# erwincoumans/tiny-differentiable-simulator

Measured on AMD Instinct MI355X. Metric: env-steps/sec, higher is better.
Workload: dtype f64

## Files before the change

### tiny-differentiable-simulator_amd/csrc/tds_oct.hip

```cpp
#include <hip/hip_runtime.h>
#include <stdlib.h>

#include "tds_device_model.h"
#include "tds_kernels.h"
#include "tds_lanes.h"
#include "tds_oct_windows.h"
#include "tds_step_shared.h"

#ifdef TDS_OCT_PROF
#ifndef TDS_OCT_PROF_WG
#define TDS_OCT_PROF_WG 3
#endif
__device__ unsigned long long tds_oct_prof_buf[64];
__device__ unsigned long long tds_oct_prof_clk[64];
__device__ unsigned long long tds_oct_prof_wg[3 * 2048];
__device__ int tds_oct_prof_iter = 500;
#define OCT_STAMP(k, pin)                                                                       \
  do {                                                                                          \
    unsigned long long t_;                                                                      \
    auto p_ = (pin);        \
    asm volatile("s_memtime %0\n\ts_waitcnt lgkmcnt(0)" : "=s"(t_), "+v"(p_)::"memory");        \
    if (prof_on) prof_t[k] = t_;                                                                \
  } while (0)
#define OCT_BAR_T(k)       \
  do {                     \
    OCT_STAMP(k, tid);     \
    OCT_BAR();             \
    OCT_STAMP((k) + 1, tid); \
  } while (0)
#define OCT_BAR_W(k, first)                                                                     \
  do {                                                                                          \
    unsigned long long a_, b_;                                                                  \
    asm volatile("s_memtime %0\n\ts_waitcnt lgkmcnt(0)" : "=s"(a_), "+v"(tid)::"memory");       \
    OCT_BAR();                                                                                  \
    asm volatile("s_memtime %0\n\ts_waitcnt lgkmcnt(0)" : "=s"(b_), "+v"(tid)::"memory");       \
    if (prof_on && (first)) {                                                                   \
      prof_t[k] = a_;                                                                           \
      prof_t[(k) + 1] = b_;                                                                     \
    } else if (prof_on) {                                                                       \
      prof_t[(k) + 2] += b_ - a_;                                                               \
    }                                                                                           \
  } while (0)
#else
#define OCT_STAMP(k, pin) do { } while (0)
#define OCT_BAR_T(k) OCT_BAR()
#define OCT_BAR_W(k, first) OCT_BAR()
#endif

#ifdef TDS_OCT_MARKS
#define OCT_MARK(name) asm volatile("; OCTMARK " name ::: "memory")
#else
#define OCT_MARK(name) do { } while (0)
#endif

namespace {

#define OCT_SYNC()                                             \
  do {                                                         \
    __builtin_amdgcn_fence(__ATOMIC_ACQ_REL, "wavefront");     \
    __builtin_amdgcn_wave_barrier();                           \
  } while (0)

template <int CTRL>
__device__ __forceinline__ double oct_dpp(double v) {
  const int l = __double2loint(v), h = __double2hiint(v);
  const int lo = __builtin_amdgcn_update_dpp(0, l, CTRL, 0xF, 0xF, true);
  const int hi = __builtin_amdgcn_update_dpp(0, h, CTRL, 0xF, 0xF, true);
  return __hiloint2double(hi, lo);
}
template <int CTRL>
__device__ __forceinline__ float oct_dpp(float v) {
  return __int_as_float(__builtin_amdgcn_update_dpp(0, __float_as_int(v), CTRL, 0xF, 0xF, true));
}
template <typename T>
__device__ __forceinline__ T pair_other(T v) { return oct_dpp<0xB1>(v); }
template <int K, typename T>
__device__ __forceinline__ T pair_bcast(T v) { return oct_dpp<(K == 0 ? 0xA0 : 0xF5)>(v); }
template <typename T>
__device__ __forceinline__ T oct_sum(T v) {
  asm volatile("" : "+v"(v));
  v += oct_dpp<0xB1>(v);
  v += oct_dpp<0x4E>(v);
  v += oct_dpp<0x141>(v);
  return v;
}
template <int K>
__device__ __forceinline__ double oct_bcast(double v) {
  const double t = __builtin_amdgcn_update_dpp(0.0, v, 0x150 + K, 0xF, 0x3, false);
  return __builtin_amdgcn_update_dpp(t, v, 0x150 + 8 + K, 0xF, 0xC, false);
}
template <int K>
__device__ __forceinline__ float oct_bcast(float v) {
  const int b = __float_as_int(v);
  const int t = __builtin_amdgcn_update_dpp(0, b, 0x150 + K, 0xF, 0x3, false);
  return __int_as_float(__builtin_amdgcn_update_dpp(t, b, 0x150 + 8 + K, 0xF, 0xC, false));
}

struct OctOff {
  int lcw, legf, swl, qdp, fac, win, xs, cp, stride;
};
struct OctLds {
  static constexpr int LCW = 6;
  static constexpr int ZW = 14;
  static constexpr int Z_B = 10, Z_A = 11, Z_G = 12, Z_HL = 13;
  static constexpr int NCP = 17;
};
__host__ __device__ inline OctOff oct_layout(int in_dim) {
  OctOff o;
  int at = in_dim + 4;
  at = (at + 1) & ~1;
  o.lcw = at;  at += 8 * OctLds::LCW;
  o.legf = at; at += 4 * 3;
  o.swl = at;  at += 8 * 6;
  o.qdp = at;  at += 8;
  o.fac = at;  at += 28;
  o.win = at;  at += 2 * 8 * OctLds::ZW;
  o.xs = at;   at += 3 * OctLds::NCP + 1;
  o.cp = at;   at += 5 * OctLds::NCP + 1;
  at = (at + 1) & ~1;
  while ((((at * 2) & 63) % 8) != 0 || ((at * 2) & 63) == 0 || ((at * 2) & 63) == 32) at += 2;
  o.stride = at;
  return o;
}

struct OctKernArgs {
  const void *mdl, *x_in;
  void *y_out;
  const void *actions;
  void *x_feedback, *obs_out;
  TdsStepCtl ctl;
  int n_envs;
  OctOff O;
};
using TB = TdsOctTab;
constexpr int TDS_OCT_PRIO = 1;

#define OCT_ST(v, p) (*(p) = (v))
#define OCT_BAR()                                                                        \
  do {                                                                                   \
    if constexpr (W2) asm volatile("s_waitcnt lgkmcnt(0)\n\ts_barrier" ::: "memory");    \
    else OCT_SYNC();                                                                     \
  } while (0)

template <typename T, typename TR, bool LOOP, int BUILD>
__device__ __forceinline__ void oct_body(const DevModel<T> *__restrict__ mdl_arg, const TR *x_in, TR *__restrict__ y_out,
                                         const TR *__restrict__ actions, TR *x_feedback ,
                                         TR *__restrict__ obs_out, const TdsStepCtl &ctl_arg, int n_envs, const OctOff &O) {
  extern __shared__ __align__(16) unsigned char tds_oct_smem[];
  T *const sm = reinterpret_cast<T *>(tds_oct_smem);
#ifdef TDS_OCT_PROF
  if (threadIdx.x == 0 && blockIdx.x < 2048) {
    unsigned long long c_;
    asm volatile("s_memrealtime %0\n\ts_waitcnt lgkmcnt(0)" : "=s"(c_)::"memory");
    tds_oct_prof_wg[3 * blockIdx.x] = c_;
  }
#endif
  constexpr bool W2 = BUILD >= 2;
  constexpr bool BATCH_SCHUR = LOOP && BUILD == 3;
  constexpr int nq = 14, nd = 14, adim = 8, in_dim = nq + nd + adim + 3, w_obs = nq + nd + 2;
  constexpr int NT = W2 ? 128 : 64;
  T *const CT = sm + 8 * O.stride;
  {
    const int t = threadIdx.x;
    constexpr int TN = (TB::TOTAL + NT - 1) / NT, XN = (in_dim + 7) / 8;
    T tv[TN], xv[XN];
#pragma unroll
    for (int k = 0; k < TN; ++k) {
      const int i = t + k * NT;
      tv[k] = i < TB::TOTAL ? mdl_arg->oct_tab[i] : T(0);
    }
    const int lane0 = t & 7, grp0 = (t & 63) >> 3, env0 = blockIdx.x * 8 + grp0;
    const bool valid0 = env0 < n_envs && t < 64;
#pragma unroll
    for (int k = 0; k < XN; ++k) {
      const int i = lane0 + 8 * k;
      const bool act = actions != nullptr && i >= nq + nd && i < nq + nd + adim;
      xv[k] = (!valid0 || i >= in_dim) ? T(0) : act ? (T)actions[(size_t)env0 * adim + (i - nq - nd)] : (T)x_in[(size_t)env0 * in_dim + i];
    }
#pragma unroll
    for (int k = 0; k < TN; ++k) {
      const int i = t + k * NT;
      if (i < TB::TOTAL) CT[i] = tv[k];
    }
    if (t < 64) {
      T *const xr = sm + grp0 * O.stride;
#pragma unroll
      for (int k = 0; k < XN; ++k) {
        const int i = lane0 + 8 * k;
        if (i < in_dim) xr[i] = xv[k];
      }
      if (lane0 < 4) xr[in_dim + lane0] = T(0);
    }
    if constexpr (W2) __syncthreads();
    else OCT_SYNC();
  }
  const int nsteps = LOOP ? ctl_arg.nsub : 1;
  T next_act = T(0);
  int act_blk = 0, y_slot = 0, o_slot = 0;
  if constexpr (LOOP) {
    if (ctl_arg.act_pool != nullptr && ctl_arg.act_blocks > 0) act_blk = (ctl_arg.act_first + 1) % ctl_arg.act_blocks;
    if (ctl_arg.y_ring != nullptr && ctl_arg.y_slots > 0) y_slot = ctl_arg.y_first % ctl_arg.y_slots;
    if (ctl_arg.obs_ring != nullptr && ctl_arg.obs_slots > 0) o_slot = ctl_arg.obs_first % ctl_arg.obs_slots;
  }
  const int act_slot = (int)(CT + (threadIdx.x & 7) * TB::LSTR)[TB::ACT];
  for (int it = 0; it < nsteps; ++it) {
  const __attribute__((address_space(4))) char *ka_seg = (const __attribute__((address_space(4))) char *)__builtin_amdgcn_kernarg_segment_ptr();
  int tid = threadIdx.x;
  if constexpr (LOOP) asm volatile("" : "+s"(ka_seg), "+v"(tid));
  const int wv = W2 ? __builtin_amdgcn_readfirstlane(tid >> 6) : 0;
  const bool is_main = !W2 || wv == 0, is_help = !W2 || wv == 1;
  if constexpr (W2 && TDS_OCT_PRIO != 0) {
    if (BUILD != 4 && wv == 0) __builtin_amdgcn_s_setprio(3);
    else __builtin_amdgcn_s_setprio(0);
  }
  (void)is_main;
  (void)is_help;
#ifdef TDS_OCT_PROF
  unsigned long long prof_t[56] = {};
  const bool prof_on = blockIdx.x == TDS_OCT_PROF_WG && it == tds_oct_prof_iter;
  if (it == 0 && tid == 0 && blockIdx.x < 2048) {
    unsigned long long c_;
    asm volatile("s_memrealtime %0\n\ts_waitcnt lgkmcnt(0)" : "=s"(c_)::"memory");
    tds_oct_prof_wg[3 * blockIdx.x + 1] = c_;
  }
  if (blockIdx.x == TDS_OCT_PROF_WG && it < 32 && tid == 0) {
    unsigned long long c0_, c1_;
    asm volatile("s_memtime %0\n\ts_memrealtime %1\n\ts_waitcnt lgkmcnt(0)" : "=s"(c0_), "=s"(c1_)::"memory");
    tds_oct_prof_clk[2 * it] = c0_;
    tds_oct_prof_clk[2 * it + 1] = c1_;
  }
#endif
  const int lane = tid & 7;
  const int grp = (tid & 63) >> 3;
  const int env = blockIdx.x * 8 + grp;
  const bool valid = env < n_envs;
  T *const E = sm + grp * O.stride;
  T *const xr = E;
  const int leg = lane >> 1, pos = lane & 1;
  const int dq = 6 + lane;
  const T *const CL = CT + lane * TB::LSTR;
  typename TdsCtlRef<LOOP>::type ctl = TdsCtlRef<LOOP>::get(ctl_arg, ka_seg + __builtin_offsetof(OctKernArgs, ctl));
  const T dt = CT[TB::SC + TB::DT];
  const int pgs_iters = (int)CT[TB::SC + TB::PGS_ITERATIONS];
  const bool last = it == nsteps - 1;
  OCT_STAMP(0, tid);

  T q, qd, tau;
  T Sl[6], R[9], p[3], sw[6], v[6], a0[6];
  T R5[9], P[3], A4[3], A5[3], pA3[3], pA4[3], pA5[3], v5[6], a5[6];
  T Lc[6], l10, id0, id1, sq0, sq1, my_id, my_sq, Ls[15], ids[6], sq_ids[6], qd_new, qdr_new[6];
  T Cb, Cr[6], It[10];
  T u = T(0), urm = T(0);
  T u_init = T(0), urm_init = T(0);
  T sw_mu = T(0), sw_rest = T(0), sw_cap = T(0), sw_hip = T(0);
  int na = 0, NA = 0;

  auto root_frame = [&](T sx, T cx, T sy, T cy, T sz, T cz) {
    R5[0] = cy * cz;                 R5[1] = -cy * sz;                R5[2] = sy;
    R5[3] = sx * sy * cz + cx * sz;  R5[4] = cx * cz - sx * sy * sz;  R5[5] = -sx * cy;
    R5[6] = sx * sz - cx * sy * cz;  R5[7] = cx * sy * sz + sx * cz;  R5[8] = cx * cy;
    P[0] = xr[0] + CT[TB::SC + TB::BASE_T];
    P[1] = xr[1] + CT[TB::SC + TB::BASE_T + 1];
    P[2] = xr[2] + CT[TB::SC + TB::BASE_T + 2];
    A4[0] = T(0); A4[1] = cx; A4[2] = sx;
    A5[0] = sy; A5[1] = -sx * cy; A5[2] = cx * cy;
    pA3[0] = T(0); pA3[1] = P[2]; pA3[2] = -P[1];
    cross3(P, A4, pA4);
    cross3(P, A5, pA5);
  };
  auto times_inertia = [&](const T *I, const T *s, T *F) {
    T t3[3];
    sym3_mulv(I, s, F);
    cross3(I + 6, s + 3, t3);
    F[0] += t3[0];
    F[1] += t3[1];
    F[2] += t3[2];
    cross3(I + 6, s, t3);
    F[3] = I[9] * s[3] - t3[0];
    F[4] = I[9] * s[4] - t3[1];
    F[5] = I[9] * s[5] - t3[2];
  };
  auto dot6 = [&](const T *a, const T *b) -> T { return dot3(a, b) + dot3(a + 3, b + 3); };

  auto main_kin = [&]() {
    OCT_MARK("main_top");
    q = xr[dq];
    qd = xr[nq + dq];
    tau = T(0);
    {
      const int act_i = act_slot;
      if (act_i >= 0) {
        const int var = nq + nd + adim;
        const T kp = xr[var], kd = xr[var + 1], max_force = xr[var + 2];
        const T act_lim = CT[TB::SC + TB::ACTION_LIMIT];
        T a = xr[nq + nd + act_i];
        a = a < act_lim ? a : act_lim;
        a = a > -act_lim ? a : -act_lim;
        const T q_des = CL[TB::IPOSE] + a;
        T f = kp * (q_des - q) + kd * (T(0) - qd);
        f = f > -max_force ? f : -max_force;
        f = f < max_force ? f : max_force;
        tau = f;
      }
      tau -= CL[TB::STIFF] * q + CL[TB::DAMP] * qd;
      asm volatile("" : "+v"(tau));
    }
    OCT_MARK("main_jcalc");
#pragma unroll
    for (int k = 0; k < 6; ++k) Sl[k] = CL[TB::S + k];
    T Rp[9], tp[3];
    {
      T sn, cs;
      tds_sincos(q * CL[TB::ROTF], &sn, &cs);
      const T c1 = T(1) - cs;
      const T nx = CL[TB::NAX], ny = CL[TB::NAX + 1], nz = CL[TB::NAX + 2];
      T RJ[9];
      RJ[0] = cs + c1 * CL[TB::NN + 0];
      RJ[1] = c1 * CL[TB::NN + 1] - sn * nz;
      RJ[2] = c1 * CL[TB::NN + 2] + sn * ny;
      RJ[3] = c1 * CL[TB::NN + 1] + sn * nz;
      RJ[4] = cs + c1 * CL[TB::NN + 3];
      RJ[5] = c1 * CL[TB::NN + 4] - sn * nx;
      RJ[6] = c1 * CL[TB::NN + 2] - sn * ny;
      RJ[7] = c1 * CL[TB::NN + 4] + sn * nx;
      RJ[8] = cs + c1 * CL[TB::NN + 5];
      const T tJ[3] = {Sl[3] * q, Sl[4] * q, Sl[5] * q};
      if (CT[TB::SC + TB::XT_IDENT] != T(0)) {
#pragma unroll
        for (int k = 0; k < 9; ++k) Rp[k] = RJ[k];
#pragma unroll
        for (int k = 0; k < 3; ++k) tp[k] = CL[TB::XT + 9 + k] + tJ[k];
      } else {
        T RT[9], r[3];
#pragma unroll
        for (int k = 0; k < 9; ++k) RT[k] = CL[TB::XT + k];
        mat3_mul(RT, RJ, Rp);
        mat3_mulv(RT, tJ, r);
#pragma unroll
        for (int k = 0; k < 3; ++k) tp[k] = CL[TB::XT + 9 + k] + r[k];
      }
    }
    OCT_MARK("main_rootsincos");
    {
      T rs, rc;
      tds_sincos(xr[3 + (lane < 3 ? lane : 0)], &rs, &rc);
      const T sx = oct_bcast<0>(rs), cx = oct_bcast<0>(rc);
      const T sy = oct_bcast<1>(rs), cy = oct_bcast<1>(rc);
      const T sz = oct_bcast<2>(rs), cz = oct_bcast<2>(rc);
      if constexpr (W2) {
        if (lane < 3) {
          T *const sc = E + O.win + 8 * OctLds::ZW + 96;
          sc[2 * lane] = rs;
          sc[2 * lane + 1] = rc;
        }
      }
      root_frame(sx, cx, sy, cy, sz, cz);
    }
    OCT_MARK("main_rootvel");
    {
      const T d0 = xr[nq + 0], d1 = xr[nq + 1], d2 = xr[nq + 2], d3 = xr[nq + 3], d4 = xr[nq + 4], d5 = xr[nq + 5];
      const T U[3] = {d0, d1, d2};
      const T J3[3] = {d3, T(0), T(0)}, J4[3] = {A4[0] * d4, A4[1] * d4, A4[2] * d4}, J5[3] = {A5[0] * d5, A5[1] * d5, A5[2] * d5};
      const T W4[3] = {J3[0] + J4[0], J3[1] + J4[1], J3[2] + J4[2]};
      const T W5[3] = {W4[0] + J5[0], W4[1] + J5[1], W4[2] + J5[2]};
      T pJ3[3], pJ4[3], pJ5[3];
      cross3(P, J3, pJ3);
      cross3(P, J4, pJ4);
      cross3(P, J5, pJ5);
      const T pW4[3] = {pJ3[0] + pJ4[0], pJ3[1] + pJ4[1], pJ3[2] + pJ4[2]};
      const T pW5[3] = {pW4[0] + pJ5[0], pW4[1] + pJ5[1], pW4[2] + pJ5[2]};
      const T V3[3] = {U[0] + pJ3[0], U[1] + pJ3[1], U[2] + pJ3[2]};
      const T V4[3] = {U[0] + pW4[0], U[1] + pW4[1], U[2] + pW4[2]};
      const T V5[3] = {U[0] + pW5[0], U[1] + pW5[1], U[2] + pW5[2]};
      T a45[3], a55[3], t1[3], t2[3], l3[3], l4[3], l5[3];
      cross3(J3, J4, a45);
      cross3(W4, J5, a55);
      cross3(J3, pJ3, t1);
      cross3(V3, J3, t2);
      l3[0] = t1[0] + t2[0]; l3[1] = t1[1] + t2[1]; l3[2] = t1[2] + t2[2];
      cross3(W4, pJ4, t1);
      cross3(V4, J4, t2);
      l4[0] = t1[0] + t2[0]; l4[1] = t1[1] + t2[1]; l4[2] = t1[2] + t2[2];
      cross3(W5, pJ5, t1);
      cross3(V5, J5, t2);
      l5[0] = t1[0] + t2[0]; l5[1] = t1[1] + t2[1]; l5[2] = t1[2] + t2[2];
#pragma unroll
      for (int k = 0; k < 3; ++k) {
        v5[k] = W5[k];
        v5[3 + k] = V5[k];
        a5[k] = a45[k] + a55[k];
        a5[3 + k] = (l3[k] + l4[k] + l5[k]) - CT[TB::SC + TB::GRAV + k];
      }
    }
    OCT_MARK("main_legs");
    {
      const bool take = pos == 1;
      T Rq[9], pq[3];
#pragma unroll
      for (int k = 0; k < 9; ++k) {
        const T sh = pair_bcast<0>(Rp[k]);
        Rq[k] = take ? sh : ((k == 0 || k == 4 || k == 8) ? T(1) : T(0));
      }
#pragma unroll
      for (int k = 0; k < 3; ++k) {
        const T sh = pair_bcast<0>(tp[k]);
        pq[k] = take ? sh : T(0);
      }
      T Rl[9], pl[3], r[3];
      mat3_mul(Rq, Rp, Rl);
      mat3_mulv(Rq, tp, r);
#pragma unroll
      for (int k = 0; k < 3; ++k) pl[k] = pq[k] + r[k];
      mat3_mul(R5, Rl, R);
      mat3_mulv(R5, pl, r);
      p[0] = P[0] + r[0];
      p[1] = P[1] + r[1];
      p[2] = P[2] + r[2];
      mat3_mulv(R, Sl, sw);
      mat3_mulv(R, Sl + 3, sw + 3);
      T c[3];
      cross3(p, sw, c);
      sw[3] += c[0];
      sw[4] += c[1];
      sw[5] += c[2];
      T vJ[6];
#pragma unroll
      for (int k = 0; k < 6; ++k) vJ[k] = sw[k] * qd;
#pragma unroll
      for (int k = 0; k < 6; ++k) {
        const T sh = pair_bcast<0>(vJ[k]);
        v[k] = v5[k] + (vJ[k] + (take ? sh : T(0)));
      }
      T cb[6];
      cross3(v, vJ, cb);
      T c1[3], c2[3];
      cross3(v, vJ + 3, c1);
      cross3(v + 3, vJ, c2);
      cb[3] = c1[0] + c2[0];
      cb[4] = c1[1] + c2[1];
      cb[5] = c1[2] + c2[2];
#pragma unroll
      for (int k = 0; k < 6; ++k) {
        const T sh = pair_bcast<0>(cb[k]);
        a0[k] = a5[k] + (cb[k] + (take ? sh : T(0)));
      }
    }
    OCT_MARK("main_publish_kin");
    {
      T *const swl = E + O.swl + lane * 6;
#pragma unroll
      for (int k = 0; k < 6; ++k) swl[k] = sw[k];
      if constexpr (W2) {
        T *const kin = E + O.win + 8 * OctLds::ZW + lane * 12;
#pragma unroll
        for (int k = 0; k < 9; ++k) kin[k] = R[k];
#pragma unroll
        for (int k = 0; k < 3; ++k) kin[9 + k] = p[k];
      }
    }
    OCT_MARK("main_kin_end");
    OCT_STAMP(1, sw[5]);
  };

  const int ystr = ctl.y_stride;
  const int out_dim = (int)CT[TB::SC + TB::OUTPUT_DIM];
  const int nv = (int)CT[TB::SC + TB::NUM_VISUALS];
  auto y_where = [&](TR *&yo, TR *&yo2, int &yend, int &yend2) {
    int ys = y_slot;
    asm volatile("" : "+s"(ys));
    yo = nullptr;
    yo2 = nullptr;
    yend = ystr;
    yend2 = out_dim;
    if (LOOP && ctl.y_ring != nullptr) {
      yo = tds_global((TR *)ctl.y_ring) + ((size_t)ys * ctl.ring_envs + env) * ystr;
      if (last && y_out != nullptr) yo2 = y_out + (size_t)env * out_dim;
    } else if (last && y_out != nullptr) {
      yo = y_out + (size_t)env * (LOOP ? out_dim : ystr);
      yend = LOOP ? out_dim : ystr;
    }
  };
  unsigned sig_tok = 0u;

  auto help_np = [&]() {
    OCT_MARK("help_np");
    if constexpr (LOOP) {
      if (it > 0 && ctl.obs_ring != nullptr && ctl.peer_arrive != nullptr)
        sig_tok = tds_peer_count_in(ctl, (o_slot == 0 ? ctl.obs_slots : o_slot) - 1);
      if (ctl.act_pool != nullptr && it + 1 < nsteps && valid)
        next_act = (T)tds_global((const TR *)ctl.act_pool)[((size_t)act_blk * ctl.act_envs + env) * adim + lane];
    }
    if constexpr (W2) {
      const T *const kin = E + O.win + 8 * OctLds::ZW + lane * 12;
#pragma unroll
      for (int k = 0; k < 9; ++k) R[k] = kin[k];
#pragma unroll
      for (int k = 0; k < 3; ++k) p[k] = kin[9 + k];
      const T *const sc = E + O.win + 8 * OctLds::ZW + 96;
      root_frame(sc[0], sc[1], sc[2], sc[3], sc[4], sc[5]);
    }
    {
      T *const cpx = E + O.cp;
      const T n[3] = {CT[TB::SC + TB::PLANE_N], CT[TB::SC + TB::PLANE_N + 1], CT[TB::SC + TB::PLANE_N + 2]};
      const T pc = CT[TB::SC + TB::PLANE_C];
      auto sphere = [&](const T *Rl, const T *pl, const T *loc, T rad, T *pt, T &dist) {
        T ctr[3];
        mat3_mulv(Rl, loc, ctr);
        ctr[0] += pl[0];
        ctr[1] += pl[1];
        ctr[2] += pl[2];
        const T t = -((-dot3(ctr, n)) + pc);
        dist = t - rad;
        pt[0] = ctr[0] - rad * n[0];
        pt[1] = ctr[1] - rad * n[1];
        pt[2] = ctr[2] - rad * n[2];
      };
      T pt0[3], pt1[3], ptt[3], d0, d1, dtt;
      sphere(R, p, CL + TB::CPL0, CL[TB::CPR0], pt0, d0);
      sphere(R, p, CL + TB::CPL1, CL[TB::CPR1], pt1, d1);
      sphere(R5, P, CT + TB::ROOT + TB::R_CPL, CT[TB::ROOT + TB::R_CPR], ptt, dtt);
      const bool act0 = valid && d0 < T(0), act1 = valid && d1 < T(0), actt = valid && dtt < T(0) && CT[TB::ROOT + TB::R_CPR] >= T(0);
      const unsigned long long b0 = __ballot(act0), b1 = __ballot(act1), bt = __ballot(actt);
      const unsigned m0 = (unsigned)((b0 >> (grp * 8)) & 0xFFull), m1 = (unsigned)((b1 >> (grp * 8)) & 0xFFull);
      const unsigned below = (1u << lane) - 1u;
      const int r0 = (actt ? 1 : 0) + __popc(m0 & below) + __popc(m1 & below);
      const int r1 = r0 + (act0 ? 1 : 0);
      if (act0) {
        cpx[0 * OctLds::NCP + r0] = pt0[0];
        cpx[1 * OctLds::NCP + r0] = pt0[1];
        cpx[2 * OctLds::NCP + r0] = pt0[2];
        cpx[3 * OctLds::NCP + r0] = d0;
        cpx[4 * OctLds::NCP + r0] = (T)lane;
      }
      if (act1) {
        cpx[0 * OctLds::NCP + r1] = pt1[0];
        cpx[1 * OctLds::NCP + r1] = pt1[1];
        cpx[2 * OctLds::NCP + r1] = pt1[2];
        cpx[3 * OctLds::NCP + r1] = d1;
        cpx[4 * OctLds::NCP + r1] = (T)lane;
      }
      if (actt && lane == 0) {
        cpx[0 * OctLds::NCP] = ptt[0];
        cpx[1 * OctLds::NCP] = ptt[1];
        cpx[2 * OctLds::NCP] = ptt[2];
        cpx[3 * OctLds::NCP] = dtt;
        cpx[4 * OctLds::NCP] = T(8);
      }
      na = (actt ? 1 : 0) + __popc(m0) + __popc(m1);
#pragma unroll
      for (int g = 0; g < 8; ++g) {
        const int c = __popc((unsigned)((b0 >> (g * 8)) & 0xFFull)) + __popc((unsigned)((b1 >> (g * 8)) & 0xFFull)) + (int)((bt >> (g * 8)) & 1ull);
        NA = c > NA ? c : NA;
      }
      if constexpr (W2) {
        if ((tid & 63) == 0) sm[in_dim + 3] = (T)NA;
      }
    }
    OCT_STAMP(8, na);
  };
  auto help_poses = [&]() {
    OCT_MARK("help_signal_poses");
    if constexpr (LOOP) {
      if (ctl.act_pool != nullptr && !last) xr[nq + nd + lane] = next_act;
      if (it > 0 && ctl.obs_ring != nullptr) {
        if (ctl.peer_arrive != nullptr) tds_peer_finish(ctl, (o_slot == 0 ? ctl.obs_slots : o_slot) - 1, sig_tok);
        else tds_signal_slot(ctl, (o_slot == 0 ? ctl.obs_slots : o_slot) - 1);
      }
    }
    TR *yo, *yo2;
    int yend, yend2;
    y_where(yo, yo2, yend, yend2);
    (void)yend;
    (void)yend2;
    if (valid && yo != nullptr && nv > 0) {
      auto pose_out = [&](const T *Rl, const T *pl, const T *vx, int k) {
        T Ro[9], po[3], qo[4];
        mat3_mul(Rl, vx, Ro);
        mat3_mulv(Rl, vx + 9, po);
        matrix_to_quat(Ro, qo);
        TR *o = yo + (nq + nd) + 7 * k;
        OCT_ST((TR)(pl[0] + po[0]), &o[0]);
        OCT_ST((TR)(pl[1] + po[1]), &o[1]);
// ... 397 lines not shown
#pragma unroll
      for (int c = 0; c < 6; ++c) {
        lch[c] = lcw[hl * OctLds::LCW + c];
        lca[c] = lcw[(hl + 1) * OctLds::LCW + c];
      }
      const T *const lf = E + O.legf + (hl >> 1) * 3;
      const T lf0 = lf[0], lf1 = lf[1], lf2 = lf[2];
      z1 -= lf0 * z0;
#pragma unroll
      for (int rr = 0; rr < 6; ++rr) rw.zr[rr] = rw.zr[rr] - (lch[rr] * z0 + lca[rr] * z1);
      rw.z0 = z0 * lf1;
      rw.z1 = z1 * lf2;
      row[0] = rw.z0;
      row[1] = rw.z1;
  };
  auto rows_park = [&](const RowRegs &rw) {
      T *const row = E + O.win + lane * OctLds::ZW;
#pragma unroll
      for (int rr = 0; rr < 6; ++rr) row[2 + rr] = rw.zr[rr];
  };
  auto rows_fetch = [&](RowRegs &rw) {
      const T *const row = E + O.win + lane * OctLds::ZW;
      rw.z0 = row[0];
      rw.z1 = row[1];
#pragma unroll
      for (int rr = 0; rr < 6; ++rr) rw.zr[rr] = row[2 + rr];
  };
  auto rows_root = [&](int bo, const RowRegs &rw) {
      OCT_MARK("rows_root");
      T *const row = E + O.win + bo + lane * OctLds::ZW;
      const T z0 = rw.z0, z1 = rw.z1;
      T zr[6];
#pragma unroll
      for (int rr = 0; rr < 6; ++rr) zr[rr] = rw.zr[rr];
      const bool real = rw.real;
      static_for<1, 6>([&](auto rc) {
        constexpr int rr = decltype(rc)::value;
        static_for<0, rr>([&](auto cc) {
          constexpr int c = decltype(cc)::value;
          zr[rr] -= Ls[(rr * (rr - 1)) / 2 + c] * zr[c];
        });
      });
#pragma unroll
      for (int rr = 0; rr < 6; ++rr) zr[rr] *= sq_ids[rr];
      const T g = ((z0 * z0 + z1 * z1) + (zr[0] * zr[0] + zr[1] * zr[1])) + ((zr[2] * zr[2] + zr[3] * zr[3]) + (zr[4] * zr[4] + zr[5] * zr[5]));
      const T ai = real ? rcp_full<T>(g + CT[TB::SC + TB::CFM]) : T(0);
#pragma unroll
      for (int rr = 0; rr < 6; ++rr) row[2 + rr] = zr[rr];
      row[OctLds::Z_A] = ai;
      row[OctLds::Z_G] = g;
      OCT_MARK("rows_root_end");
      OCT_STAMP(10, ai);
  };
  auto main_sweep = [&](auto firstc, int w0, int bo, bool lw) {
      constexpr bool FIRST = decltype(firstc)::value;
      constexpr int KMAX = (FIRST && W2) ? 12 : 8;
      OCT_MARK("sweep");
      const T *const Zs = E + O.win + bo;
      T *const xw = E + O.xs + w0;
      const T my_hip = sw_hip, mu = sw_mu, rest = sw_rest;
      const int wn = 3 * NA - w0, k_n = NA - w0, k_t2 = 2 * NA - w0;
      const T *const xs1 = xw - NA, *const xs2 = xw - 2 * NA;
      struct Ops { T zs, zm, b, a, g, hl, sd, xo; };
      auto request = [&](auto kc, Ops &o) {
        constexpr int k = decltype(kc)::value;
        const T *const row = Zs + k * OctLds::ZW;
        o.zs = row[pos];
        o.zm = row[2 + lane];
        o.b = row[OctLds::Z_B];
        o.a = row[OctLds::Z_A];
        o.hl = row[OctLds::Z_HL];
        if constexpr (!FIRST) {
          o.g = row[OctLds::Z_G];
          o.xo = xw[k];
        }
      };
      auto process = [&](auto kc, const Ops &o, auto normalc) {
        constexpr int k = decltype(kc)::value;
        constexpr bool NORMAL = decltype(normalc)::value;
        const T zl = o.hl == my_hip ? o.zs : T(0);
        T jw;
        if constexpr (NORMAL) jw = oct_sum(zl * (u + rest * u_init) + o.zm * (urm + rest * urm_init));
        else jw = oct_sum(zl * u + o.zm * urm);
        T xn;
        if constexpr (FIRST) xn = (o.b - jw) * o.a;
        else xn = (o.b - (jw - o.g * o.xo)) * o.a;
        if constexpr (NORMAL) {
          xn = max_t<T>(xn, T(0));
          xn = min_t<T>(xn, sw_cap);
        } else {
          const T hi = mu * max_t<T>(o.sd, T(0));
          xn = max_t<T>(xn, -hi);
          xn = min_t<T>(xn, hi);
        }
        T dx;
        if constexpr (FIRST) dx = xn;
        else dx = xn - o.xo;
        u += zl * dx;
        urm += o.zm * dx;
        xw[k] = xn;
      };
      Ops ops[2];
      auto rows = [&](auto self, auto kc) -> void {
        constexpr int k = decltype(kc)::value;
        if constexpr (k < 8) {
          if (k >= wn) return;
          Ops &cur = ops[k & 1];
          if constexpr (k < 7) request(std::integral_constant<int, k + 1>{}, ops[(k + 1) & 1]);
          if (k < k_n) {
            process(kc, cur, std::true_type{});
          } else {
            cur.sd = (k >= k_t2 ? xs2 : xs1)[k];
            if constexpr (k == 7 && KMAX > 8) {
              if (lw) {
                OCT_BAR_W(30, false);
                request(std::integral_constant<int, 8>{}, ops[0]);
              }
            }
            process(kc, cur, std::false_type{});
          }
          self(self, std::integral_constant<int, k + 1>{});
        } else if constexpr (k < KMAX) {
          if (k == 8 ? !lw : k >= wn) return;
          Ops &cur = ops[k & 1];
          if constexpr (k + 1 < KMAX) request(std::integral_constant<int, k + 1>{}, ops[(k + 1) & 1]);
          cur.sd = xs2[k];
          process(kc, cur, std::false_type{});
          self(self, std::integral_constant<int, k + 1>{});
        }
      };
      request(std::integral_constant<int, 0>{}, ops[0]);
      rows(rows, std::integral_constant<int, 0>{});
      OCT_SYNC();
      OCT_MARK("sweep_end");
  };

  bool done_reg = false, done_in_reg = false;
  auto main_fin = [&]() {
    OCT_MARK("main_fin");
    OCT_STAMP(6, u);
    {
      T w = u * my_sq;
      T wr[6];
      static_for<0, 6>([&](auto rc) {
        constexpr int r = decltype(rc)::value;
        wr[r] = oct_bcast<r>(urm) * sq_ids[r];
      });
      static_for<0, 5>([&](auto ic) {
        constexpr int r = 4 - decltype(ic)::value;
        static_for<r + 1, 6>([&](auto cc) {
          constexpr int c = decltype(cc)::value;
          wr[r] -= Ls[(c * (c - 1)) / 2 + r] * wr[c];
        });
      });
#pragma unroll
      for (int r = 0; r < 6; ++r) w -= Lc[r] * wr[r];
      w -= (pos == 0 ? l10 : T(0)) * pair_bcast<1>(w);
      qd_new = qd - w;
#pragma unroll
      for (int r = 0; r < 6; ++r) qdr_new[r] = xr[nq + r] - wr[r];
    }
    OCT_MARK("main_integrate");
    T qn0, qn2, qo0;
    const int rm = (int)CT[TB::SC + TB::REWARD_MODE];
    const T inv_dt = CT[TB::SC + TB::INV_DT];
    OCT_SYNC();
    {
      T qn_root[6];
#pragma unroll
      for (int r = 0; r < 6; ++r) qn_root[r] = xr[r] + qdr_new[r] * dt;
      const T q_old0 = xr[0];
      qn0 = qn_root[0];
      qn2 = qn_root[2];
      qo0 = q_old0;
      OCT_SYNC();
      if (lane == 0) {
#pragma unroll
        for (int r = 0; r < 6; ++r) {
          xr[r] = qn_root[r];
          xr[nq + r] = qdr_new[r];
        }
      }
      xr[dq] = q + qd_new * dt;
      xr[nq + dq] = qd_new;
      if (lane == 0) {
        xr[in_dim] = q_old0;
        xr[in_dim + 3] = T(0);
      }
    }
    OCT_SYNC();
    OCT_MARK("main_reward");
    done_in_reg = rm == TDS_REWARD_ANT;
    if (rm == TDS_REWARD_ANT) {
      const T vel_x = (qn0 - qo0) * inv_dt;
      done_reg = qn2 < T(0.26);
      const T reward = done_reg ? T(0) : vel_x;
      if (lane == 0) {
        xr[in_dim + 1] = done_reg ? T(1) : T(0);
        xr[in_dim + 2] = reward;
      }
    } else {
      T rs = T(0), rc = T(1);
      if (rm == TDS_REWARD_LAIKAGO) sincos_t<T>(lane < 3 ? xr[3 + lane] * T(0.5) : T(0), &rs, &rc);
      const T s1 = oct_bcast<1>(rs), c1 = oct_bcast<1>(rc), s2 = oct_bcast<2>(rs), c2 = oct_bcast<2>(rc);
      if (lane == 0) {
        bool done = false;
        T reward = T(0);
        if (rm == TDS_REWARD_LAIKAGO) {
          const T sp = rs, cp = rc, st = s1, ct = c1, ss = s2, cs2 = c2;
          const T qx = sp * ct * cs2 - cp * st * ss;
          const T qy = cp * st * cs2 + sp * ct * ss;
          const T qz = cp * ct * ss - sp * st * cs2;
          const T qw = cp * ct * cs2 + sp * st * ss;
          const T sq = T(2) / (qx * qx + qy * qy + qz * qz + qw * qw);
          const T up = T(1) - (qx * (qx * sq) + qy * (qy * sq));
          done = (up < T(0.6)) || (xr[2] < T(0.2));
          reward = done ? T(0) : xr[0];
        }
        xr[in_dim + 1] = done ? T(1) : T(0);
        xr[in_dim + 2] = reward;
      }
    }
    OCT_SYNC();
  };
  auto y_state = [&](TR *y, int end) {
    {
      constexpr int NB = (nq + nd + 7) / 8;
      T sv[NB];
#pragma unroll
      for (int k = 0; k < NB; ++k) sv[k] = xr[lane + 8 * k < nq + nd ? lane + 8 * k : 0];
#pragma unroll
      for (int k = 0; k < NB; ++k)
        if (lane + 8 * k < nq + nd) OCT_ST((TR)sv[k], &y[lane + 8 * k]);
    }
    int tail = nq + nd;
    if ((int)CT[TB::SC + TB::PACK_VISUALS]) {
      tail += 7 * nv;
      if (lane == 0) OCT_ST((TR)(CT[TB::SC + TB::BASE_R8]), &y[tail]);
      tail += 1;
    }
    for (int i = tail + lane; i < end; i += 8) OCT_ST(TR(0), &y[i]);
  };
  auto main_pool = [&]() {
    OCT_MARK("main_pool");
    if (ctl.pool != nullptr && valid && (done_in_reg ? done_reg : xr[in_dim + 1] != T(0))) {
      TR *yo, *yo2;
      int yend, yend2;
      y_where(yo, yo2, yend, yend2);
      if (yo != nullptr) {
        y_state(yo, yend);
        if (yo2 != nullptr) y_state(yo2, yend2);
      }
      const unsigned c = ctl.reset_count[env];
      const TR *const src = tds_global((const TR *)ctl.pool) + ((size_t)(c % (unsigned)ctl.pool_depth) * ctl.pool_envs + env) * (nq + nd);
      T v0 = (T)src[lane], v1 = (T)src[lane + 8], v2 = (T)src[lane + 16], v3 = T(0);
      if (lane + 24 < nq + nd) v3 = (T)src[lane + 24];
      OCT_SYNC();
      xr[lane] = v0;
      xr[lane + 8] = v1;
      xr[lane + 16] = v2;
      if (lane + 24 < nq + nd) xr[lane + 24] = v3;
      if (lane == 0) {
        ctl.reset_count[env] = c + 1u;
        xr[in_dim + 3] = T(1);
      }
    }
    OCT_MARK("main_pool_end");
    OCT_STAMP(7, tid);
  };
  auto help_rec = [&]() {
    OCT_MARK("help_rec");
    TR *yo, *yo2;
    int yend, yend2;
    y_where(yo, yo2, yend, yend2);
    if (valid && yo != nullptr && xr[in_dim + 3] == T(0)) {
      y_state(yo, yend);
      if (yo2 != nullptr) y_state(yo2, yend2);
    }
    if constexpr (LOOP) {
      if (ctl.obs_ring != nullptr) {
        const int slot = o_slot;
        const int rf = ctl.ring_flags;
        const bool f32w = (rf & TDS_RING_OBS_F32) != 0 || sizeof(TR) == 4;
        const int np = ctl.peer_arrive != nullptr ? ctl.n_peers : 0;
        const bool rd_only = (rf & TDS_RING_PEER_REWARD_DONE) != 0;
        if (ctl.peer_arrive != nullptr && (rf & TDS_RING_WIDE) != 0 && __all(valid)) {
          const int wl = tid & 63;
          const size_t row0 = ((size_t)slot * ctl.obs_envs + (size_t)blockIdx.x * 8) * (size_t)w_obs;
          const int per_unit = f32w ? 2 : 1;
          const int n_units = (8 * w_obs) / per_unit;
          const unsigned long long *const __attribute__((address_space(4))) *tab =
              (const unsigned long long *const __attribute__((address_space(4))) *)(const __attribute__((address_space(4))) void *)ctl.peer_ring;
          for (int u0 = 0; u0 < n_units; u0 += 64) {
            const int uu = u0 + wl;
            const bool on = uu < n_units;
            unsigned lo = 0u, hi = 0u;
            bool tail = false;
#pragma unroll
            for (int c = 0; c < 2; ++c) {
              if (c < per_unit) {
                const int f = on ? uu * per_unit + c : 0;
                const int e = f / w_obs;
                const int i = f - e * w_obs;
                const int src = i < nq + nd ? i : (i == nq + nd ? in_dim + 2 : in_dim + 1);
                const T vv = i < 2 ? T(0) : sm[e * O.stride + src];
                tail = tail || i >= nq + nd;
                if (f32w) {
                  const unsigned b = (unsigned)__float_as_int((float)vv);
                  if (c == 0) lo = b; else hi = b;
                } else {
                  const double dv = (double)vv;
                  lo = (unsigned)__double2loint(dv);
                  hi = (unsigned)__double2hiint(dv);
                }
              }
            }
            const unsigned long long bits = ((unsigned long long)hi << 32) | (unsigned long long)lo;
            const size_t unit_at = row0 / per_unit + (size_t)uu;
            if (on) __hip_atomic_store(tds_global((unsigned long long *)ctl.obs_ring) + unit_at, bits, __ATOMIC_RELAXED, __HIP_MEMORY_SCOPE_AGENT);
            const bool to_peers = on && (!rd_only || tail);
            for (int p0 = 0; p0 < np; p0 += 4) {
              const unsigned long long *const b0 = tds_global(tab[p0]), *const b1 = tds_global(tab[p0 + 1]), *const b2 = tds_global(tab[p0 + 2]),
                                       *const b3 = tds_global(tab[p0 + 3]);
              const size_t po = (size_t)ctl.peer_off / 8 + unit_at;
              if (to_peers) {
                using G64 = __attribute__((address_space(1))) unsigned long long;
                __hip_atomic_store((G64 *)((unsigned long long *)b0 + po), bits, __ATOMIC_RELAXED, __HIP_MEMORY_SCOPE_SYSTEM);
                if (p0 + 1 < np) __hip_atomic_store((G64 *)((unsigned long long *)b1 + po), bits, __ATOMIC_RELAXED, __HIP_MEMORY_SCOPE_SYSTEM);
                if (p0 + 2 < np) __hip_atomic_store((G64 *)((unsigned long long *)b2 + po), bits, __ATOMIC_RELAXED, __HIP_MEMORY_SCOPE_SYSTEM);
                if (p0 + 3 < np) __hip_atomic_store((G64 *)((unsigned long long *)b3 + po), bits, __ATOMIC_RELAXED, __HIP_MEMORY_SCOPE_SYSTEM);
              }
            }
          }
        } else if (valid) {
          const size_t at = ((size_t)slot * ctl.obs_envs + env) * w_obs;
          constexpr int NB = (w_obs + 7) / 8;
          T ov[NB];
#pragma unroll
          for (int k = 0; k < NB; ++k) {
            const int i = lane + 8 * k;
            const T rv = xr[i >= w_obs ? 0 : (i < nq + nd ? i : (i == nq + nd ? in_dim + 2 : in_dim + 1))];
            ov[k] = i < 2 ? T(0) : rv;
          }
#pragma unroll
          for (int k = 0; k < NB; ++k) {
            const int i = lane + 8 * k;
            if (i >= w_obs) continue;
// ... 67 lines not shown
      OCT_BAR_T(40);
      help_np();
      RowRegs rw = {};
      if (NA > 0) rows_geom(0, 0, rw);
      OCT_BAR_T(42);
      if (NA > 0) {
        rows_leg(0, rw);
        rows_park(rw);
      }
      help_poses();
      if (NA > 0) rows_fetch(rw);
      OCT_BAR_T(44);
      if (tds_oct_help_has_windows(NA, pgs_iters)) {
        help_get_factors();
        rows_root(0, rw);
        OCT_BAR_W(46, true);
        const int nr = 3 * NA;
        int bo = 8 * OctLds::ZW;
        for (int pit = 0; pit < pgs_iters; ++pit) {
          for (int w0 = tds_oct_help_first_w0(pit); w0 < nr; w0 += 8) {
            rows_geom(w0, bo, rw);
            rows_leg(bo, rw);
            rows_root(bo, rw);
            OCT_BAR_W(46, false);
            bo = 8 * OctLds::ZW - bo;
          }
        }
      }
      OCT_BAR_T(50);
      help_rec();
    }
  } else {
    main_kin();
    OCT_SYNC();
    help_np();
    help_poses();
    main_dyn();
    OCT_SYNC();
    main_dyn2();
    main_fd();
    main_sweep_consts();
    const int nr = 3 * NA;
    int bo = 0;
    for (int pit = 0; pit < pgs_iters; ++pit) {
      for (int w0 = 0; w0 < nr; w0 += 8) {
        RowRegs rw;
        rows_geom(w0, bo, rw);
        rows_leg(bo, rw);
        rows_root(bo, rw);
        OCT_SYNC();
        if (pit == 0) main_sweep(std::true_type{}, w0, bo, false);
        else main_sweep(std::false_type{}, w0, bo, false);
        bo = 8 * OctLds::ZW - bo;
      }
    }
    main_fin();
    main_pool();
    OCT_SYNC();
    help_rec();
    if constexpr (LOOP) OCT_SYNC();
  }
#ifdef TDS_OCT_PROF
  if (prof_on && (tid & 63) == 0) {
#pragma unroll
    for (int k = 16; k < 24; ++k)
      if (is_main) tds_oct_prof_buf[k] = prof_t[k];
#pragma unroll
    for (int k = 0; k < 14; ++k)
      if (((k < 8 || k >= 12) && is_main) || (k >= 8 && k < 12 && is_help)) tds_oct_prof_buf[k] = prof_t[k];
    if (is_help) tds_oct_prof_buf[15] = (unsigned long long)NA;
#pragma unroll
    for (int k = 24; k < 36; ++k)
      if (is_main) tds_oct_prof_buf[k] = prof_t[k];
#pragma unroll
    for (int k = 40; k < 52; ++k)
      if (is_help) tds_oct_prof_buf[k] = prof_t[k];
  }
#endif
  if constexpr (LOOP) {
    act_blk = act_blk + 1 >= ctl_arg.act_blocks ? 0 : act_blk + 1;
    y_slot = y_slot + 1 >= ctl_arg.y_slots ? 0 : y_slot + 1;
    o_slot = o_slot + 1 >= ctl_arg.obs_slots ? 0 : o_slot + 1;
  }
  }
#ifdef TDS_OCT_PROF
  if (threadIdx.x == 0 && blockIdx.x < 2048) {
    unsigned long long c_;
    asm volatile("s_waitcnt vmcnt(0)\n\ts_memrealtime %0\n\ts_waitcnt lgkmcnt(0)" : "=s"(c_)::"memory");
    tds_oct_prof_wg[3 * blockIdx.x + 2] = c_;
  }
#endif
}

template <typename T, typename TR, bool LOOP, int BUILD>
__global__ __launch_bounds__(BUILD >= 2 ? 128 : 64) __attribute__((amdgpu_waves_per_eu(BUILD == 2 ? 2 : 1, BUILD == 2 ? 2 : 1)))
void tds_oct_kernel(const DevModel<T> *__restrict__ mdl_arg, const TR *x_in, TR *__restrict__ y_out,
                    const TR *__restrict__ actions, TR *x_feedback, TR *__restrict__ obs_out, TdsStepCtl ctl_arg, int n_envs,
                    OctOff O) {
  oct_body<T, TR, LOOP, BUILD>(mdl_arg, x_in, y_out, actions, x_feedback, obs_out, ctl_arg, n_envs, O);
}
template <typename T, typename TR, bool LOOP>
__global__ __launch_bounds__(128) __attribute__((amdgpu_waves_per_eu(2, 2), amdgpu_num_vgpr(120)))
void tds_oct_kernel_beside(const DevModel<T> *__restrict__ mdl_arg, const TR *x_in, TR *__restrict__ y_out,
                           const TR *__restrict__ actions, TR *x_feedback, TR *__restrict__ obs_out, TdsStepCtl ctl_arg,
                           int n_envs, OctOff O) {
  oct_body<T, TR, LOOP, 4>(mdl_arg, x_in, y_out, actions, x_feedback, obs_out, ctl_arg, n_envs, O);
}

}

#ifdef TDS_OCT_PROF
extern "C" int tds_oct_prof_workgroups(unsigned long long *out, int n_wg) {
  return hipMemcpyFromSymbol(out, HIP_SYMBOL(tds_oct_prof_wg), (size_t)3 * n_wg * sizeof(unsigned long long)) == hipSuccess ? 0 : -1;
}
extern "C" int tds_oct_prof_clocks(unsigned long long *out64) {
  return hipMemcpyFromSymbol(out64, HIP_SYMBOL(tds_oct_prof_clk), 64 * sizeof(unsigned long long)) == hipSuccess ? 0 : -1;
}
extern "C" int tds_oct_prof_read(unsigned long long *out64, int iter) {
  if (out64 && hipMemcpyFromSymbol(out64, HIP_SYMBOL(tds_oct_prof_buf), 64 * sizeof(unsigned long long)) != hipSuccess) return -1;
  if (iter >= 0 && hipMemcpyToSymbol(HIP_SYMBOL(tds_oct_prof_iter), &iter, sizeof(int)) != hipSuccess) return -1;
  return 0;
}
#endif

int tds_oct_lds_bytes(int input_dim) { return oct_layout(input_dim).stride * (int)sizeof(double); }
int tds_oct_workgroup_bytes(int input_dim) {
  return (oct_layout(input_dim).stride * 8 + TdsOctTab::TOTAL) * (int)sizeof(double);
}

template <typename T, typename TR>
int tds_launch_oct(const DevModel<T> *d_model, const DevModel<T> &h_model, const TR *x_in, TR *y_out, const TR *actions,
                   TR *x_feedback, TR *obs_out, int n_envs, hipStream_t stream, const TdsStepCtl &ctl, int build) {
  const OctOff O = oct_layout(h_model.input_dim);
  const int blocks = (n_envs + 7) / 8;
  const size_t shmem = ((size_t)O.stride * 8 + TdsOctTab::TOTAL) * sizeof(T);
  const bool one_step = ctl.nsub == 1 && ctl.obs_ring == nullptr && ctl.y_ring == nullptr;
#define OCT_LAUNCH(LOOP_, B_)                                                                                                 \
  hipLaunchKernelGGL((tds_oct_kernel<T, TR, LOOP_, B_>), dim3(blocks), dim3(B_ >= 2 ? 128 : 64), shmem, stream, d_model, x_in, \
                     y_out, actions, x_feedback, obs_out, ctl, n_envs, O)
  if (build == 4) {
    if (one_step)
      hipLaunchKernelGGL((tds_oct_kernel_beside<T, TR, false>), dim3(blocks), dim3(128), shmem, stream, d_model, x_in, y_out, actions,
                         x_feedback, obs_out, ctl, n_envs, O);
    else
      hipLaunchKernelGGL((tds_oct_kernel_beside<T, TR, true>), dim3(blocks), dim3(128), shmem, stream, d_model, x_in, y_out, actions,
                         x_feedback, obs_out, ctl, n_envs, O);
  } else if (one_step) {
    if (build == 3) OCT_LAUNCH(false, 3);
    else if (build == 2) OCT_LAUNCH(false, 2);
    else OCT_LAUNCH(false, 1);
  } else {
    if (build == 3) OCT_LAUNCH(true, 3);
    else if (build == 2) OCT_LAUNCH(true, 2);
    else OCT_LAUNCH(true, 1);
  }
#undef OCT_LAUNCH
  return (int)hipGetLastError();
}
template int tds_launch_oct<double, double>(const DevModel<double> *, const DevModel<double> &, const double *, double *,
                                            const double *, double *, double *, int, hipStream_t, const TdsStepCtl &, int);
template int tds_launch_oct<double, float>(const DevModel<double> *, const DevModel<double> &, const float *, float *,
                                           const float *, float *, float *, int, hipStream_t, const TdsStepCtl &, int);
```

Before: 628.9 million.

## Carry joint state in registers, prefetch constants early, split loop per wave role

The per-step body becomes a lambda templated on wave role, so the BUILD 3 loop can be instantiated separately for the main and helper waves with the role known at compile time. The joint and root state (q, qd, root pose and velocity) is carried in registers across iterations instead of being re-read from LDS, and is reloaded only when an env is reset from the pool. Per-lane model constants and gains are fetched before the end-of-step sync so their LDS latency is hidden. An asm barrier also delays use of the friction bound in the PGS loop. These changes raise register pressure and duplicate the code for each role, which can hurt occupancy or instruction-cache behaviour.

After: 654.8 million (median of 6 runs). 1.04x the previous value.

```diff
diff --git a/tiny-differentiable-simulator_amd/csrc/tds_oct.hip b/tiny-differentiable-simulator_amd/csrc/tds_oct.hip
--- a/tiny-differentiable-simulator_amd/csrc/tds_oct.hip
+++ b/tiny-differentiable-simulator_amd/csrc/tds_oct.hip
@@ -53,6 +53,19 @@
 #define OCT_MARK(name) do { } while (0)
 #endif
 
+#ifndef TDS_OCT_SD_LATE
+#define TDS_OCT_SD_LATE 1
+#endif
+#ifndef TDS_OCT_CARRY
+#define TDS_OCT_CARRY 1
+#endif
+#ifndef TDS_OCT_TOP_EARLY
+#define TDS_OCT_TOP_EARLY 1
+#endif
+#ifndef TDS_OCT_SPLIT_LOOP
+#define TDS_OCT_SPLIT_LOOP 0
+#endif
+
 namespace {
 
 #define OCT_SYNC()                                             \
@@ -157,6 +170,10 @@
 #endif
   constexpr bool W2 = BUILD >= 2;
   constexpr bool BATCH_SCHUR = LOOP && BUILD == 3;
+  constexpr bool SD_LATE = LOOP && (BUILD == 2 || BUILD == 3) && TDS_OCT_SD_LATE != 0;
+  constexpr bool CARRY = LOOP && BUILD == 3 && TDS_OCT_CARRY != 0;
+  constexpr bool TOP_EARLY = LOOP && BUILD == 3 && TDS_OCT_TOP_EARLY != 0;
+  constexpr bool SPLIT_LOOP = CARRY || TOP_EARLY || (LOOP && BUILD == 3 && TDS_OCT_SPLIT_LOOP != 0);
   constexpr int nq = 14, nd = 14, adim = 8, in_dim = nq + nd + adim + 3, w_obs = nq + nd + 2;
   constexpr int NT = W2 ? 128 : 64;
   T *const CT = sm + 8 * O.stride;
@@ -203,11 +220,55 @@
     if (ctl_arg.obs_ring != nullptr && ctl_arg.obs_slots > 0) o_slot = ctl_arg.obs_first % ctl_arg.obs_slots;
   }
   const int act_slot = (int)(CT + (threadIdx.x & 7) * TB::LSTR)[TB::ACT];
-  for (int it = 0; it < nsteps; ++it) {
+  struct Carried { T q, qd, rq[6], rqd[6]; };
+  struct TopConsts { T S[6], rotf, nax[3], nn[6], xt[3], ipose, stiff, damp, act_lim, xt_ident, base_t[3], grav[3], kp, kd, max_force; };
+  auto carry_load = [&](const T *xr_, int lane_, Carried &c) {
+    c.q = xr_[6 + lane_];
+    c.qd = xr_[nq + 6 + lane_];
+#pragma unroll
+    for (int r = 0; r < 6; ++r) {
+      c.rq[r] = xr_[r];
+      c.rqd[r] = xr_[nq + r];
+    }
+  };
+  auto top_request = [&](const T *xr_, const T *CL_, TopConsts &t) {
+#pragma unroll
+    for (int k = 0; k < 6; ++k) t.S[k] = CL_[TB::S + k];
+    t.rotf = CL_[TB::ROTF];
+#pragma unroll
+    for (int k = 0; k < 3; ++k) t.nax[k] = CL_[TB::NAX + k];
+#pragma unroll
+    for (int k = 0; k < 6; ++k) t.nn[k] = CL_[TB::NN + k];
+#pragma unroll
+    for (int k = 0; k < 3; ++k) t.xt[k] = CL_[TB::XT + 9 + k];
+    t.ipose = CL_[TB::IPOSE];
+    t.stiff = CL_[TB::STIFF];
+    t.damp = CL_[TB::DAMP];
+    t.act_lim = CT[TB::SC + TB::ACTION_LIMIT];
+    t.xt_ident = CT[TB::SC + TB::XT_IDENT];
+#pragma unroll
+    for (int k = 0; k < 3; ++k) {
+      t.base_t[k] = CT[TB::SC + TB::BASE_T + k];
+      t.grav[k] = CT[TB::SC + TB::GRAV + k];
+    }
+    t.kp = xr_[nq + nd + adim];
+    t.kd = xr_[nq + nd + adim + 1];
+    t.max_force = xr_[nq + nd + adim + 2];
+  };
+  Carried car = {};
+  TopConsts tc = {};
+  if constexpr (CARRY || TOP_EARLY) {
+    const int lane_ = threadIdx.x & 7;
+    const T *const xr_ = sm + ((threadIdx.x & 63) >> 3) * O.stride;
+    if constexpr (CARRY) carry_load(xr_, lane_, car);
+    if constexpr (TOP_EARLY) top_request(xr_, CT + lane_ * TB::LSTR, tc);
+  }
+  auto step_body = [&](auto rolec, const int it) {
+  constexpr int ROLE = decltype(rolec)::value;
   const __attribute__((address_space(4))) char *ka_seg = (const __attribute__((address_space(4))) char *)__builtin_amdgcn_kernarg_segment_ptr();
   int tid = threadIdx.x;
   if constexpr (LOOP) asm volatile("" : "+s"(ka_seg), "+v"(tid));
-  const int wv = W2 ? __builtin_amdgcn_readfirstlane(tid >> 6) : 0;
+  const int wv = ROLE < 2 ? ROLE : (W2 ? __builtin_amdgcn_readfirstlane(tid >> 6) : 0);
   const bool is_main = !W2 || wv == 0, is_help = !W2 || wv == 1;
   if constexpr (W2 && TDS_OCT_PRIO != 0) {
     if (BUILD != 4 && wv == 0) __builtin_amdgcn_s_setprio(3);
@@ -255,13 +316,13 @@
   T sw_mu = T(0), sw_rest = T(0), sw_cap = T(0), sw_hip = T(0);
   int na = 0, NA = 0;
 
-  auto root_frame = [&](T sx, T cx, T sy, T cy, T sz, T cz) {
+  auto root_frame = [&](const T *rq, const T *bt, T sx, T cx, T sy, T cy, T sz, T cz) {
     R5[0] = cy * cz;                 R5[1] = -cy * sz;                R5[2] = sy;
     R5[3] = sx * sy * cz + cx * sz;  R5[4] = cx * cz - sx * sy * sz;  R5[5] = -sx * cy;
     R5[6] = sx * sz - cx * sy * cz;  R5[7] = cx * sy * sz + sx * cz;  R5[8] = cx * cy;
-    P[0] = xr[0] + CT[TB::SC + TB::BASE_T];
-    P[1] = xr[1] + CT[TB::SC + TB::BASE_T + 1];
-    P[2] = xr[2] + CT[TB::SC + TB::BASE_T + 2];
+    P[0] = rq[0] + bt[0];
+    P[1] = rq[1] + bt[1];
+    P[2] = rq[2] + bt[2];
     A4[0] = T(0); A4[1] = cx; A4[2] = sx;
     A5[0] = sy; A5[1] = -sx * cy; A5[2] = cx * cy;
     pA3[0] = T(0); pA3[1] = P[2]; pA3[2] = -P[1];
@@ -284,52 +345,58 @@
 
   auto main_kin = [&]() {
     OCT_MARK("main_top");
-    q = xr[dq];
-    qd = xr[nq + dq];
+#define OCT_TOP(early, read) (TOP_EARLY ? (early) : (read))
+    if constexpr (CARRY) {
+      q = car.q;
+      qd = car.qd;
+    } else {
+      q = xr[dq];
+      qd = xr[nq + dq];
+    }
     tau = T(0);
     {
       const int act_i = act_slot;
       if (act_i >= 0) {
         const int var = nq + nd + adim;
-        const T kp = xr[var], kd = xr[var + 1], max_force = xr[var + 2];
-        const T act_lim = CT[TB::SC + TB::ACTION_LIMIT];
+        const T kp = OCT_TOP(tc.kp, xr[var]), kd = OCT_TOP(tc.kd, xr[var + 1]), max_force = OCT_TOP(tc.max_force, xr[var + 2]);
+        const T act_lim = OCT_TOP(tc.act_lim, CT[TB::SC + TB::ACTION_LIMIT]);
         T a = xr[nq + nd + act_i];
         a = a < act_lim ? a : act_lim;
         a = a > -act_lim ? a : -act_lim;
-        const T q_des = CL[TB::IPOSE] + a;
+        const T q_des = OCT_TOP(tc.ipose, CL[TB::IPOSE]) + a;
         T f = kp * (q_des - q) + kd * (T(0) - qd);
         f = f > -max_force ? f : -max_force;
         f = f < max_force ? f : max_force;
         tau = f;
       }
-      tau -= CL[TB::STIFF] * q + CL[TB::DAMP] * qd;
+      tau -= OCT_TOP(tc.stiff, CL[TB::STIFF]) * q + OCT_TOP(tc.damp, CL[TB::DAMP]) * qd;
       asm volatile("" : "+v"(tau));
     }
     OCT_MARK("main_jcalc");
 #pragma unroll
-    for (int k = 0; k < 6; ++k) Sl[k] = CL[TB::S + k];
+    for (int k = 0; k < 6; ++k) Sl[k] = OCT_TOP(tc.S[k], CL[TB::S + k]);
     T Rp[9], tp[3];
     {
       T sn, cs;
-      tds_sincos(q * CL[TB::ROTF], &sn, &cs);
+      tds_sincos(q * OCT_TOP(tc.rotf, CL[TB::ROTF]), &sn, &cs);
       const T c1 = T(1) - cs;
-      const T nx = CL[TB::NAX], ny = CL[TB::NAX + 1], nz = CL[TB::NAX + 2];
+      const T nx = OCT_TOP(tc.nax[0], CL[TB::NAX]), ny = OCT_TOP(tc.nax[1], CL[TB::NAX + 1]), nz = OCT_TOP(tc.nax[2], CL[TB::NAX + 2]);
       T RJ[9];
-      RJ[0] = cs + c1 * CL[TB::NN + 0];
-      RJ[1] = c1 * CL[TB::NN + 1] - sn * nz;
-      RJ[2] = c1 * CL[TB::NN + 2] + sn * ny;
-      RJ[3] = c1 * CL[TB::NN + 1] + sn * nz;
-      RJ[4] = cs + c1 * CL[TB::NN + 3];
-      RJ[5] = c1 * CL[TB::NN + 4] - sn * nx;
-      RJ[6] = c1 * CL[TB::NN + 2] - sn * ny;
-      RJ[7] = c1 * CL[TB::NN + 4] + sn * nx;
-      RJ[8] = cs + c1 * CL[TB::NN + 5];
+      RJ[0] = cs + c1 * OCT_TOP(tc.nn[0], CL[TB::NN + 0]);
+      RJ[1] = c1 * OCT_TOP(tc.nn[1], CL[TB::NN + 1]) - sn * nz;
+      RJ[2] = c1 * OCT_TOP(tc.nn[2], CL[TB::NN + 2]) + sn * ny;
+      RJ[3] = c1 * OCT_TOP(tc.nn[1], CL[TB::NN + 1]) + sn * nz;
+      RJ[4] = cs + c1 * OCT_TOP(tc.nn[3], CL[TB::NN + 3]);
+      RJ[5] = c1 * OCT_TOP(tc.nn[4], CL[TB::NN + 4]) - sn * nx;
+      RJ[6] = c1 * OCT_TOP(tc.nn[2], CL[TB::NN + 2]) - sn * ny;
+      RJ[7] = c1 * OCT_TOP(tc.nn[4], CL[TB::NN + 4]) + sn * nx;
+      RJ[8] = cs + c1 * OCT_TOP(tc.nn[5], CL[TB::NN + 5]);
       const T tJ[3] = {Sl[3] * q, Sl[4] * q, Sl[5] * q};
-      if (CT[TB::SC + TB::XT_IDENT] != T(0)) {
+      if (OCT_TOP(tc.xt_ident, CT[TB::SC + TB::XT_IDENT]) != T(0)) {
 #pragma unroll
         for (int k = 0; k < 9; ++k) Rp[k] = RJ[k];
 #pragma unroll
-        for (int k = 0; k < 3; ++k) tp[k] = CL[TB::XT + 9 + k] + tJ[k];
+        for (int k = 0; k < 3; ++k) tp[k] = OCT_TOP(tc.xt[k], CL[TB::XT + 9 + k]) + tJ[k];
       } else {
         T RT[9], r[3];
 #pragma unroll
@@ -337,13 +404,20 @@
         mat3_mul(RT, RJ, Rp);
         mat3_mulv(RT, tJ, r);
 #pragma unroll
-        for (int k = 0; k < 3; ++k) tp[k] = CL[TB::XT + 9 + k] + r[k];
+        for (int k = 0; k < 3; ++k) tp[k] = OCT_TOP(tc.xt[k], CL[TB::XT + 9 + k]) + r[k];
       }
     }
     OCT_MARK("main_rootsincos");
     {
       T rs, rc;
-      tds_sincos(xr[3 + (lane < 3 ? lane : 0)], &rs, &rc);
+      T ang;
+      if constexpr (CARRY) {
+        const T a3 = car.rq[3], a4 = car.rq[4], a5 = car.rq[5];
+        ang = lane == 1 ? a4 : (lane == 2 ? a5 : a3);
+      } else {
+        ang = xr[3 + (lane < 3 ? lane : 0)];
+      }
+      tds_sincos(ang, &rs, &rc);
       const T sx = oct_bcast<0>(rs), cx = oct_bcast<0>(rc);
       const T sy = oct_bcast<1>(rs), cy = oct_bcast<1>(rc);
       const T sz = oct_bcast<2>(rs), cz = oct_bcast<2>(rc);
@@ -354,11 +428,12 @@
           sc[2 * lane + 1] = rc;
         }
       }
-      root_frame(sx, cx, sy, cy, sz, cz);
+      root_frame(CARRY ? car.rq : xr, TOP_EARLY ? tc.base_t : CT + TB::SC + TB::BASE_T, sx, cx, sy, cy, sz, cz);
     }
     OCT_MARK("main_rootvel");
     {
-      const T d0 = xr[nq + 0], d1 = xr[nq + 1], d2 = xr[nq + 2], d3 = xr[nq + 3], d4 = xr[nq + 4], d5 = xr[nq + 5];
+      const T *const rqd = CARRY ? car.rqd : xr + nq;
+      const T d0 = rqd[0], d1 = rqd[1], d2 = rqd[2], d3 = rqd[3], d4 = rqd[4], d5 = rqd[5];
       const T U[3] = {d0, d1, d2};
       const T J3[3] = {d3, T(0), T(0)}, J4[3] = {A4[0] * d4, A4[1] * d4, A4[2] * d4}, J5[3] = {A5[0] * d5, A5[1] * d5, A5[2] * d5};
       const T W4[3] = {J3[0] + J4[0], J3[1] + J4[1], J3[2] + J4[2]};
@@ -389,9 +464,10 @@
         v5[k] = W5[k];
         v5[3 + k] = V5[k];
         a5[k] = a45[k] + a55[k];
-        a5[3 + k] = (l3[k] + l4[k] + l5[k]) - CT[TB::SC + TB::GRAV + k];
-      }
-    }
+        a5[3 + k] = (l3[k] + l4[k] + l5[k]) - OCT_TOP(tc.grav[k], CT[TB::SC + TB::GRAV + k]);
+      }
+    }
+#undef OCT_TOP
     OCT_MARK("main_legs");
     {
       const bool take = pos == 1;
@@ -497,7 +573,7 @@
 #pragma unroll
       for (int k = 0; k < 3; ++k) p[k] = kin[9 + k];
       const T *const sc = E + O.win + 8 * OctLds::ZW + 96;
-      root_frame(sc[0], sc[1], sc[2], sc[3], sc[4], sc[5]);
+      root_frame(xr, CT + TB::SC + TB::BASE_T, sc[0], sc[1], sc[2], sc[3], sc[4], sc[5]);
     }
     {
       T *const cpx = E + O.cp;
@@ -1061,6 +1137,11 @@
         T jw;
         if constexpr (NORMAL) jw = oct_sum(zl * (u + rest * u_init) + o.zm * (urm + rest * urm_init));
         else jw = oct_sum(zl * u + o.zm * urm);
+        T sd = T(0);
+        if constexpr (!NORMAL) {
+          sd = o.sd;
+          if constexpr (SD_LATE) asm volatile("" : "+v"(jw), "+v"(sd));
+        }
         T xn;
         if constexpr (FIRST) xn = (o.b - jw) * o.a;
         else xn = (o.b - (jw - o.g * o.xo)) * o.a;
@@ -1068,7 +1149,7 @@
           xn = max_t<T>(xn, T(0));
           xn = min_t<T>(xn, sw_cap);
         } else {
-          const T hi = mu * max_t<T>(o.sd, T(0));
+          const T hi = mu * max_t<T>(sd, T(0));
           xn = max_t<T>(xn, -hi);
           xn = min_t<T>(xn, hi);
         }
@@ -1152,6 +1233,7 @@
       qn0 = qn_root[0];
       qn2 = qn_root[2];
       qo0 = q_old0;
+      if constexpr (TOP_EARLY) top_request(xr, CL, tc);
       OCT_SYNC();
       if (lane == 0) {
 #pragma unroll
@@ -1160,8 +1242,18 @@
           xr[nq + r] = qdr_new[r];
         }
       }
-      xr[dq] = q + qd_new * dt;
+      const T q_new = q + qd_new * dt;
+      xr[dq] = q_new;
       xr[nq + dq] = qd_new;
+      if constexpr (CARRY) {
+        car.q = q_new;
+        car.qd = qd_new;
+#pragma unroll
+        for (int r = 0; r < 6; ++r) {
+          car.rq[r] = qn_root[r];
+          car.rqd[r] = qdr_new[r];
+        }
+      }
       if (lane == 0) {
         xr[in_dim] = q_old0;
         xr[in_dim + 3] = T(0);
@@ -1222,7 +1314,8 @@
   };
   auto main_pool = [&]() {
     OCT_MARK("main_pool");
-    if (ctl.pool != nullptr && valid && (done_in_reg ? done_reg : xr[in_dim + 1] != T(0))) {
+    const bool replaced = ctl.pool != nullptr && valid && (done_in_reg ? done_reg : xr[in_dim + 1] != T(0));
+    if (replaced) {
       TR *yo, *yo2;
       int yend, yend2;
       y_where(yo, yo2, yend, yend2);
@@ -1242,6 +1335,12 @@
       if (lane == 0) {
         ctl.reset_count[env] = c + 1u;
         xr[in_dim + 3] = T(1);
+      }
+    }
+    if constexpr (CARRY) {
+      if (ctl.pool != nullptr && __any(replaced)) {
+        OCT_SYNC();
+        carry_load(xr, lane, car);
       }
     }
     OCT_MARK("main_pool_end");
@@ -1475,6 +1574,15 @@
     y_slot = y_slot + 1 >= ctl_arg.y_slots ? 0 : y_slot + 1;
     o_slot = o_slot + 1 >= ctl_arg.obs_slots ? 0 : o_slot + 1;
   }
+  };
+  if constexpr (SPLIT_LOOP) {
+    if (__builtin_amdgcn_readfirstlane((int)threadIdx.x >> 6) == 0) {
+      for (int it = 0; it < nsteps; ++it) step_body(std::integral_constant<int, 0>{}, it);
+    } else {
+      for (int it = 0; it < nsteps; ++it) step_body(std::integral_constant<int, 1>{}, it);
+    }
+  } else {
+    for (int it = 0; it < nsteps; ++it) step_body(std::integral_constant<int, 2>{}, it);
   }
 #ifdef TDS_OCT_PROF
   if (threadIdx.x == 0 && blockIdx.x < 2048) {
```
